# LDeakin/zarrs_tools

Hardware: AMD Instinct MI355X
Metric: GiB/s filtered (device-resident), guided_filter r=4, 2048³ f32, 256³ chunks (higher is better)
Workload: dtype f32; 1 GPU; guided_filter eps=2500 r=4 on a 2048x2048x2048 f32 array, 256^3 chunks, device-resident; rank g owns a z-slab of chunk rows + 2r halo; chunks_total=512, chunks_rank0=512, parallelism=chunk-rows x1 (strong)

## Files before the change

### zarrs_tools_amd/csrc/gf_fused.hpp

```cpp
#pragma once

#include <hip/hip_runtime.h>

#include <atomic>
#include <stdint.h>

#include <algorithm>
#include <type_traits>

#include "zt_device.hpp"
#include "zt_kernels.hpp"

#ifndef GF_K4_R4
#define GF_K4_R4 8
#endif
#ifndef GF_ORDER_R4
#define GF_ORDER_R4 2
#endif
#ifndef GF_ORDER
#define GF_ORDER 0
#endif
#ifndef GF_PRIO
#define GF_PRIO 1
#endif
#ifndef GF_HX_B128
#define GF_HX_B128 1
#endif
#ifndef GF_P1RING_MAXR
#define GF_P1RING_MAXR 2
#endif
#ifndef GF_K3
#define GF_K3 4
#endif
#ifndef GF_K4
#define GF_K4 4
#endif
#ifndef GF_STX
#define GF_STX 4
#endif
#ifndef GF_STY
#define GF_STY 16
#endif
#ifndef GF_P1PFD
#define GF_P1PFD 2
#endif
#ifndef GF_P1PFD_R4M1
#define GF_P1PFD_R4M1 1
#endif
#ifndef GF_P1PFD_R2
#define GF_P1PFD_R2 2
#endif
#ifndef GF_CNTREG
#define GF_CNTREG 1
#endif
#ifndef GF_P3VPF
#define GF_P3VPF 2
#endif
#ifndef GF_P5VPF
#define GF_P5VPF 1
#endif
#ifndef GF_WAVE_SKIP
#define GF_WAVE_SKIP 1
#endif

namespace zt {

template <int R, int K>
__device__ __forceinline__ void tree_window_sums(const float (&in)[K + 2 * R], float (&out)[K]) {
    constexpr int W = 2 * R + 1;
    if constexpr (W == 1) {
#pragma unroll
        for (int i = 0; i < K; ++i) out[i] = in[i];
    } else {
        constexpr int N = K + 2 * R;
        float p2[N], p4[N], p8[N], p16[N], p32[N], p64[N], p128[N];
#pragma unroll
        for (int i = 0; i + 1 < N; ++i) p2[i] = in[i] + in[i + 1];
        if constexpr (W >= 4) {
#pragma unroll
            for (int i = 0; i + 3 < N; ++i) p4[i] = p2[i] + p2[i + 2];
        }
        if constexpr (W >= 8) {
#pragma unroll
            for (int i = 0; i + 7 < N; ++i) p8[i] = p4[i] + p4[i + 4];
        }
        if constexpr (W >= 16) {
#pragma unroll
            for (int i = 0; i + 15 < N; ++i) p16[i] = p8[i] + p8[i + 8];
        }
        if constexpr (W >= 32) {
#pragma unroll
            for (int i = 0; i + 31 < N; ++i) p32[i] = p16[i] + p16[i + 16];
        }
        if constexpr (W >= 64) {
#pragma unroll
            for (int i = 0; i + 63 < N; ++i) p64[i] = p32[i] + p32[i + 32];
        }
        if constexpr (W >= 128) {
#pragma unroll
            for (int i = 0; i + 127 < N; ++i) p128[i] = p64[i] + p64[i + 64];
        }
#pragma unroll
        for (int i = 0; i < K; ++i) {
            float acc = 0.0f;
            int off = 0;
            bool first = true;
#pragma unroll
            for (int b = 7; b >= 0; --b) {
                if (W & (1 << b)) {
                    float piece;
                    switch (b) {
                    case 0: piece = in[i + off]; break;
                    case 1: piece = p2[i + off]; break;
                    case 2: piece = p4[i + off]; break;
                    case 3: piece = p8[i + off]; break;
                    case 4: piece = p16[i + off]; break;
                    case 5: piece = p32[i + off]; break;
                    case 6: piece = p64[i + off]; break;
                    default: piece = p128[i + off]; break;
                    }
                    acc = first ? piece : acc + piece;
                    first = false;
                    off += 1 << b;
                }
            }
            out[i] = acc;
        }
    }
}

template <int R, int K, typename T>
__device__ __forceinline__ void tree_window_sums_t(const T (&in)[K + 2 * R], T (&out)[K]) {
    constexpr int W = 2 * R + 1;
    constexpr int N = K + 2 * R;
    if constexpr (W == 1) {
#pragma unroll
        for (int i = 0; i < K; ++i) out[i] = in[i];
    } else {
        T p2[N], p4[N], p8[N], p16[N];
#pragma unroll
        for (int i = 0; i + 1 < N; ++i) p2[i] = in[i] + in[i + 1];
        if constexpr (W >= 4) {
#pragma unroll
            for (int i = 0; i + 3 < N; ++i) p4[i] = p2[i] + p2[i + 2];
        }
        if constexpr (W >= 8) {
#pragma unroll
            for (int i = 0; i + 7 < N; ++i) p8[i] = p4[i] + p4[i + 4];
        }
        if constexpr (W >= 16) {
#pragma unroll
            for (int i = 0; i + 15 < N; ++i) p16[i] = p8[i] + p8[i + 8];
        }
        static_assert(W < 32, "fused radii only");
#pragma unroll
        for (int i = 0; i < K; ++i) {
            T acc{};
            int off = 0;
            bool first = true;
#pragma unroll
            for (int b = 4; b >= 0; --b) {
                if (W & (1 << b)) {
                    T piece;
                    switch (b) {
                    case 0: piece = in[i + off]; break;
                    case 1: piece = p2[i + off]; break;
                    case 2: piece = p4[i + off]; break;
                    case 3: piece = p8[i + off]; break;
                    default: piece = p16[i + off]; break;
                    }
                    acc = first ? piece : acc + piece;
                    first = false;
                    off += 1 << b;
                }
            }
            out[i] = acc;
        }
    }
}


typedef float f2 __attribute__((ext_vector_type(2)));

__device__ __forceinline__ f2 pk_fma(f2 a, f2 b, f2 c) { return __builtin_elementwise_fma(a, b, c); }

template <int R, int K, typename T>
__device__ __forceinline__ void core_window_sums(const T (&in)[K + 2 * R], T (&out)[K]);

__device__ __forceinline__ int clamped_count(int i, int n, int r) {
    int lo = i - r < 0 ? 0 : i - r;
    int hi = i + r > n - 1 ? n - 1 : i + r;
    return hi - lo + 1;
}
__device__ __forceinline__ int cmul(int a, int b) { return (int)__umul24((unsigned)a, (unsigned)b); }

template <int R, int K, typename T>
__device__ __forceinline__ void core_window_sums(const T (&in)[K + 2 * R], T (&out)[K]) {
    constexpr int W = 2 * R + 1;
    if constexpr (K > W || K < 2) {
        tree_window_sums_t<R, K>(in, out);
    } else {
        constexpr int NC = W - K + 1;
        T c[NC];
#pragma unroll
        for (int j = 0; j < NC; ++j) c[j] = in[K - 1 + j];
#pragma unroll
        for (int w = 1; w < NC; w *= 2) {
#pragma unroll
            for (int j = 0; j + w < NC; j += 2 * w) c[j] = c[j] + c[j + w];
        }
        const T core = c[0];
        T left[K], right[K];
        if constexpr (K >= 2) {
            left[K - 2] = in[K - 2];
#pragma unroll
            for (int i = K - 3; i >= 0; --i) left[i] = in[i] + left[i + 1];
            right[1] = in[W];
#pragma unroll
            for (int i = 2; i < K; ++i) right[i] = right[i - 1] + in[W + i - 1];
        }
        out[0] = left[0] + core;
#pragma unroll
        for (int i = 1; i < K - 1; ++i) out[i] = (left[i] + core) + right[i];
        out[K - 1] = core + right[K - 1];
    }
}

template <int B, int E, typename F>
__device__ __forceinline__ void static_for(F&& f) {
    if constexpr (B < E) {
        f(std::integral_constant<int, B>{});
        static_for<B + 1, E>(f);
    }
}

template <int S, int W>
struct RingDispatch {
    template <typename F>
    __device__ __forceinline__ static void run(int slot, F&& f) {
        if (slot == S) f(std::integral_constant<int, S>{});
        else RingDispatch<S + 1, W>::run(slot, f);
    }
};
template <int W>
struct RingDispatch<W, W> {
    template <typename F>
    __device__ __forceinline__ static void run(int, F&&) {}
};

template <int R, int K, typename T>
__device__ __forceinline__ void slide_sums_exact(const T (&in)[K + 2 * R], T (&out)[K]) {
    T c[2 * R + 1];
#pragma unroll
    for (int j = 0; j <= 2 * R; ++j) c[j] = in[j];
#pragma unroll
    for (int w = 1; w <= 2 * R; w *= 2) {
#pragma unroll
        for (int j = 0; j + w <= 2 * R; j += 2 * w) c[j] = c[j] + c[j + w];
    }
    T d[K];
#pragma unroll
    for (int i = 1; i < K; ++i) d[i] = in[i + 2 * R] - in[i - 1];
    out[0] = c[0];
#pragma unroll
    for (int i = 1; i < K; ++i) out[i] = out[i - 1] + d[i];
}

template <typename T> struct S1 {
    using acc = double;
    using in = float;
    static constexpr int HXB = 8;
};
template <> struct S1<uint8_t> { using acc = int; using in = int; static constexpr int HXB = 4; };
template <> struct S1<uint16_t> { using acc = int; using in = int; static constexpr int HXB = 4; };

__device__ __forceinline__ float fast_div(float x, float d) {
    float y = __builtin_amdgcn_rcpf(d);
    float e = __builtin_fmaf(-d, y, 1.0f);
    y = __builtin_fmaf(e, y, y);
    float q = x * y;
    float r = __builtin_fmaf(-d, q, x);
    return __builtin_fmaf(r, y, q);
}

__device__ __forceinline__ void lds_barrier() {
    __asm__ volatile("s_waitcnt lgkmcnt(0)\n\ts_barrier" ::: "memory");
}

__device__ __forceinline__ float div_by_count(float x, float d, float rcp) {
    float q = x * rcp;
    float r = __builtin_fmaf(-q, d, x);
    return __builtin_fmaf(r, rcp, q);
}

using rsrc_t = __amdgpu_buffer_rsrc_t;
#ifndef GF_OUT_AUX
#define GF_OUT_AUX 2
#endif
constexpr int kBadOff = (int)0x80000000;

__device__ __forceinline__ rsrc_t make_rsrc(const void* base, uint32_t bytes) {
    return __builtin_amdgcn_make_buffer_rsrc(const_cast<void*>(base), (short)0, (int)bytes,
                                             0x00020000);
}

template <typename T> struct Buf;
template <> struct Buf<float> {
    template <int AUX = 0>
    __device__ static float load(rsrc_t r, int off) {
        return __builtin_bit_cast(float, __builtin_amdgcn_raw_buffer_load_b32(r, off, 0, AUX));
    }
    __device__ static void store(float v, rsrc_t r, int off) {
        __builtin_amdgcn_raw_buffer_store_b32(__builtin_bit_cast(uint32_t, v), r, off, 0, GF_OUT_AUX);
    }
};
template <> struct Buf<uint16_t> {
    template <int AUX = 0>
    __device__ static float load(rsrc_t r, int off) {
        return (float)(uint16_t)__builtin_amdgcn_raw_buffer_load_b16(r, off, 0, AUX);
    }
    __device__ static int load_int(rsrc_t r, int off) {
        return (int)(uint16_t)__builtin_amdgcn_raw_buffer_load_b16(r, off, 0, 0);
    }
    __device__ static void store(uint16_t v, rsrc_t r, int off) {
        __builtin_amdgcn_raw_buffer_store_b16(v, r, off, 0, 2);
    }
};
template <> struct Buf<uint8_t> {
    template <int AUX = 0>
    __device__ static float load(rsrc_t r, int off) {
        return (float)(uint8_t)__builtin_amdgcn_raw_buffer_load_b8(r, off, 0, AUX);
    }
    __device__ static int load_int(rsrc_t r, int off) {
        return (int)(uint8_t)__builtin_amdgcn_raw_buffer_load_b8(r, off, 0, 0);
    }
    __device__ static void store(uint8_t v, rsrc_t r, int off) {
        __builtin_amdgcn_raw_buffer_store_b8(v, r, off, 0, 2);
    }
};

__device__ __forceinline__ double dpp_from_lower(double v) {
    const int lo = __builtin_amdgcn_mov_dpp(__double2loint(v), 0x138, 0xF, 0xF, true);
    const int hi = __builtin_amdgcn_mov_dpp(__double2hiint(v), 0x138, 0xF, 0xF, true);
    return __hiloint2double(hi, lo);
}
__device__ __forceinline__ double dpp_from_upper(double v) {
    const int lo = __builtin_amdgcn_mov_dpp(__double2loint(v), 0x130, 0xF, 0xF, true);
    const int hi = __builtin_amdgcn_mov_dpp(__double2hiint(v), 0x130, 0xF, 0xF, true);
    return __hiloint2double(hi, lo);
}
__device__ __forceinline__ int dpp_from_lower(int v) {
    return __builtin_amdgcn_mov_dpp(v, 0x138, 0xF, 0xF, true);
}
__device__ __forceinline__ int dpp_from_upper(int v) {
    return __builtin_amdgcn_mov_dpp(v, 0x130, 0xF, 0xF, true);
}

typedef unsigned int u32x4 __attribute__((ext_vector_type(4)));
typedef unsigned int u32x2 __attribute__((ext_vector_type(2)));

template <typename T> struct Quad;
template <> struct Quad<float> {
    template <int AUX = 0>
    __device__ static void load(rsrc_t r, int off, float (&v)[4]) {
        const u32x4 q = __builtin_amdgcn_raw_buffer_load_b128(r, off, 0, AUX);
        v[0] = __uint_as_float(q.x); v[1] = __uint_as_float(q.y);
        v[2] = __uint_as_float(q.z); v[3] = __uint_as_float(q.w);
    }
    __device__ static void store(const float (&v)[4], rsrc_t r, int off) {
        const u32x4 q = {__float_as_uint(v[0]), __float_as_uint(v[1]), __float_as_uint(v[2]),
                         __float_as_uint(v[3])};
        __builtin_amdgcn_raw_buffer_store_b128(q, r, off, 0, GF_OUT_AUX);
    }
};
template <> struct Quad<uint16_t> {
    template <int AUX = 0>
    __device__ static void load(rsrc_t r, int off, float (&v)[4]) {
        const u32x2 q = __builtin_amdgcn_raw_buffer_load_b64(r, off, 0, AUX);
        v[0] = (float)(q.x & 0xffffu); v[1] = (float)(q.x >> 16);
        v[2] = (float)(q.y & 0xffffu); v[3] = (float)(q.y >> 16);
    }
    __device__ static void load(rsrc_t r, int off, int (&v)[4]) {
        const u32x2 q = __builtin_amdgcn_raw_buffer_load_b64(r, off, 0, 0);
        v[0] = (int)(q.x & 0xffffu); v[1] = (int)(q.x >> 16);
        v[2] = (int)(q.y & 0xffffu); v[3] = (int)(q.y >> 16);
    }
    __device__ static void store(const float (&v)[4], rsrc_t r, int off) {
        const uint32_t a = (uint32_t)from_f32<uint16_t>(v[0]) | ((uint32_t)from_f32<uint16_t>(v[1]) << 16);
        const uint32_t b = (uint32_t)from_f32<uint16_t>(v[2]) | ((uint32_t)from_f32<uint16_t>(v[3]) << 16);
        __builtin_amdgcn_raw_buffer_store_b64((u32x2){a, b}, r, off, 0, 2);
    }
};
template <> struct Quad<uint8_t> {
    template <int AUX = 0>
    __device__ static void load(rsrc_t r, int off, float (&v)[4]) {
        const uint32_t q = __builtin_amdgcn_raw_buffer_load_b32(r, off, 0, AUX);
        v[0] = (float)(q & 0xffu); v[1] = (float)((q >> 8) & 0xffu);
        v[2] = (float)((q >> 16) & 0xffu); v[3] = (float)(q >> 24);
    }
    __device__ static void load(rsrc_t r, int off, int (&v)[4]) {
        const uint32_t q = __builtin_amdgcn_raw_buffer_load_b32(r, off, 0, 0);
        v[0] = (int)(q & 0xffu); v[1] = (int)((q >> 8) & 0xffu);
        v[2] = (int)((q >> 16) & 0xffu); v[3] = (int)(q >> 24);
    }
    __device__ static void store(const float (&v)[4], rsrc_t r, int off) {
        const uint32_t a = (uint32_t)from_f32<uint8_t>(v[0]) | ((uint32_t)from_f32<uint8_t>(v[1]) << 8) |
                           ((uint32_t)from_f32<uint8_t>(v[2]) << 16) | ((uint32_t)from_f32<uint8_t>(v[3]) << 24);
        __builtin_amdgcn_raw_buffer_store_b32(a, r, off, 0, 2);
    }
};

__device__ __forceinline__ int opaque(int v) {
    __asm__ volatile("" : "+v"(v));
    return v;
}

template <typename T>
__device__ __forceinline__ void load_quad_masked(rsrc_t r, int off, int mask, float (&v)[4]) {
#pragma unroll
    for (int e = 0; e < 4; ++e)
        v[e] = Buf<T>::load(r, (mask >> e) & 1 ? off + e * (int)sizeof(T) : kBadOff);
}
template <typename T>
__device__ __forceinline__ void load_quad_masked(rsrc_t r, int off, int mask, int (&v)[4]) {
#pragma unroll
    for (int e = 0; e < 4; ++e)
        v[e] = Buf<T>::load_int(r, (mask >> e) & 1 ? off + e * (int)sizeof(T) : kBadOff);
}
template <typename T>
__device__ __forceinline__ void store_quad_masked(const float (&v)[4], rsrc_t r, int off, int mask) {
#pragma unroll
    for (int e = 0; e < 4; ++e)
        Buf<T>::store(from_f32<T>(v[e]), r, (mask >> e) & 1 ? off + e * (int)sizeof(T) : kBadOff);
}

template <int R, int TY, int NT, int HXB = 8>
struct GFConfig {
    static constexpr int TX = 64;
    static constexpr int W = 2 * R + 1;
    static constexpr int HXB_ = HXB;
    static constexpr int E2X = TX + 4 * R, E2Y = TY + 4 * R;
    static constexpr int E1X = TX + 2 * R, E1Y = TY + 2 * R;
    static constexpr int p2m4(int x) { return x + ((2 - x % 4) + 4) % 4; }
    static constexpr int ph4(int x) { return (x + 3) / 4 * 4 + ((x + 3) / 4 * 4 % 8 == 0 ? 4 : 0); }
    static constexpr int PH = HXB == 8 ? p2m4(E1X) : ph4(E1X);
    static constexpr int PA = p2m4(E1X);
    static constexpr int PB = p2m4(TX);
    static constexpr bool R4 = R == 4 && TY == 32 && NT == 1024;
    static constexpr int K3 = GF_K3, K4 = R4 ? GF_K4_R4 : GF_K4;
    static constexpr int ORDER = R4 ? GF_ORDER_R4 : GF_ORDER;
    static constexpr int K5 = TX * TY / NT;
    static constexpr int S3 = (E1Y + K3 - 1) / K3;
    static constexpr int S4 = TX / K4;
    static constexpr int N3 = E1X * S3, N4 = E1Y * S4;
    static constexpr int QPL = 1;
    static constexpr int EPL = 4 * QPL;
    static constexpr int NQ1X = E2X / EPL;
    static constexpr int RPW = 64 / NQ1X;
    static constexpr int NWAVE = NT / 64;
    static constexpr int NQP1 = (E2Y + RPW * NWAVE - 1) / (RPW * NWAVE);
    static constexpr int W12 = NQP1 == 1 ? NWAVE - (E2Y + RPW - 1) / RPW : 0;
    static constexpr int NB = (R + EPL - 1) / EPL;
    static constexpr bool P1RING = R <= GF_P1RING_MAXR;
    static constexpr int NQ5 = TX / 4 * TY;
    static constexpr int W3 = W * W * W;
    static constexpr int al(int b) { return (b + 255) / 256 * 256; }
    static constexpr int SZ_HX = al((E2Y + K3) * PH * HXB);
    static constexpr int SZ_LAB = al((E1Y + 1) * PA * 8);
    static constexpr int SZ_HAB = al((E1Y + 1) * PB * 8);
    static constexpr int SZ_RCP = al((W3 + 1) * 4);
    static constexpr int OFF_HX = 0, OFF_LAB = OFF_HX + SZ_HX;
    static constexpr int OFF_HAB = OFF_LAB + SZ_LAB;
    static constexpr int OFF_RCP = OFF_HAB + SZ_HAB;
    static constexpr int LDS_BYTES = OFF_RCP + SZ_RCP;
    static constexpr int T3 = NT - N3;
    static_assert(TX * TY % NT == 0, "tile must divide evenly over the threads");
    static_assert(TY % K5 == 0, "ring segment must divide the tile height");
    static_assert(TX % K4 == 0, "P4 segment must divide the tile width");
    static_assert(N3 <= NT && N4 <= NT, "one work item per thread per phase");
    static_assert(RPW >= 1, "an E2 row fits one wave");
    static_assert(E2X % 4 == 0, "E2 rows are whole quads");
    static_assert(E2X % EPL == 0, "E2 rows are whole lane items");
    static_assert(LDS_BYTES <= 160 * 1024, "LDS budget");
};

template <int R, int TY, int NT, typename TIn, typename TOut, int MODE>
__global__ __launch_bounds__(NT) void gf3d_fused_kernel(GFParams p) {
    using C = GFConfig<R, TY, NT, S1<TIn>::HXB>;
    using SA = typename S1<TIn>::acc;
    using SI = typename S1<TIn>::in;
    constexpr bool EDGE = MODE == 2, INTERIOR = MODE == 0;
    constexpr int TX = C::TX, W = C::W;
    constexpr int K5 = C::K5;
    constexpr int ESZ = (int)sizeof(TIn), OSZ = (int)sizeof(TOut);
    extern __shared__ __attribute__((aligned(16))) char smem[];
    SA* const Hx = reinterpret_cast<SA*>(smem + C::OFF_HX);
    float2* const Lab = reinterpret_cast<float2*>(smem + C::OFF_LAB);
    float2* const Hab = reinterpret_cast<float2*>(smem + C::OFF_HAB);
    float* const rcp_tab = reinterpret_cast<float*>(smem + C::OFF_RCP);
    for (int c = threadIdx.x; c <= C::W3; c += NT) rcp_tab[c] = c > 0 ? 1.0f / (float)c : 0.0f;

    const int nwg = gridDim.x;
    const int b = blockIdx.x;
    const int lid = (nwg % 8 == 0) ? (b % 8) * (nwg / 8) + b / 8 : b;
    const int gtx = INTERIOR ? p.itx1 - p.itx0 : p.tiles_x;
    const int gty = INTERIOR ? p.ity1 - p.ity0 : p.tiles_y;
    const int ntiles = gtx * gty;
    const int seg = lid / ntiles;
    int t = lid % ntiles;
    int tile_x, tile_y;
    {
        const int stx = GF_STX, sty = GF_STY;
        const int full_y = gty / sty * sty;
        const int per_srow = gtx * sty;
        if (t < full_y * gtx) {
            const int sr = t / per_srow, r = t % per_srow;
            const int full_x = gtx / stx * stx;
            if (r < full_x * sty) {
                tile_x = (r / (stx * sty)) * stx + r % stx;
                tile_y = sr * sty + (r / stx) % sty;
            } else {
                const int rr = r - full_x * sty, w = gtx - full_x;
                tile_x = full_x + rr % w;
                tile_y = sr * sty + rr / w;
            }
        } else {
            t -= full_y * gtx;
            tile_x = t % gtx;
            tile_y = full_y + t / gtx;
        }
    }
    if constexpr (INTERIOR) {
        tile_x += p.itx0;
        tile_y += p.ity0;
    } else {
        if (tile_x >= p.itx0 && tile_x < p.itx1 && tile_y >= p.ity0 && tile_y < p.ity1) return;
    }

    const int x0 = p.ox0 + tile_x * TX;
    const int y0 = p.oy0 + tile_y * TY;
    const int ox_end = p.ox0 + p.onx, oy_end = p.oy0 + p.ony;
    const int zo_begin = p.oz0 + seg * p.zseg;
    const int zo_end = min(zo_begin + p.zseg, p.oz0 + p.onz);
    const int nz = p.nz, ny = p.ny, nx = p.nx;
    const float eps = p.eps;
    const uint32_t slice_bytes = (uint32_t)((int64_t)(p.ny - 1) * p.in_sy + p.nx) * ESZ;
    const uint32_t oslice_bytes =
        (uint32_t)((int64_t)(p.ony - 1) * p.out_sy + p.onx) * OSZ;
    const int sy = (int)p.in_sy, osy = (int)p.out_sy;

    const char* in_base = static_cast<const char*>(p.in);
    const int zlo = p.zlo, zspan = p.zhi - p.zlo;
    auto slice_rsrc = [&](int z) -> rsrc_t {
        const bool ok = (unsigned)(z - zlo) < (unsigned)zspan;
        const char* base = in_base + (ok ? (int64_t)(z - p.in_z0) * p.in_sz * ESZ : 0);
        return make_rsrc(base, ok ? slice_bytes : 0u);
    };

    const int zc_begin = zo_begin - R, zc_end = zo_end + R;

    const int tid0 = threadIdx.x;
    constexpr int EPL = C::EPL;
    int q1off[C::NQP1], q1mask[C::NQP1];
    auto p12_pos = [&](int tid, int k, int& row, int& cq) -> bool {
        const int w = tid / 64 - C::W12, l = tid % 64;
        row = (k * C::NWAVE + w) * C::RPW + l / C::NQ1X;
        cq = l % C::NQ1X;
        return w >= 0 && l < C::RPW * C::NQ1X && row < C::E2Y;
    };
#pragma unroll
    for (int k = 0; k < C::NQP1; ++k) {
        int row, cq;
        const bool valid = p12_pos(tid0, k, row, cq);
        const int gx = x0 - 2 * R + EPL * cq, gy = y0 - 2 * R + row;
        int m = 0;
        if (valid && gy >= 0 && gy < ny) {
#pragma unroll
            for (int e = 0; e < 4; ++e) m |= (gx + e >= 0 && gx + e < nx) ? (1 << e) : 0;
        }
        q1mask[k] = m;
        q1off[k] = (EDGE ? valid : m == 0xF) ? (gy * sy + gx) * ESZ : kBadOff;
    }
    auto load_quad = [&](rsrc_t r, int off, int mask, SI (&v)[4]) {
        if constexpr (EDGE) load_quad_masked<TIn>(r, off, mask, v);
        else Quad<TIn>::load(r, off, v);
    };

    SA zv[C::NQP1][EPL];
#pragma unroll
    for (int k = 0; k < C::NQP1; ++k)
#pragma unroll
        for (int e = 0; e < EPL; ++e) zv[k][e] = (SA)0;
    SI ring1[C::P1RING ? W : 1][C::NQP1][EPL];
    if constexpr (C::P1RING) {
        static_for<0, W>([&](auto jc) {
            constexpr int j = decltype(jc)::value;
            const rsrc_t rs = slice_rsrc(zc_begin - 1 - R + j);
#pragma unroll
            for (int k = 0; k < C::NQP1; ++k) {
                SI v[4];
                load_quad(rs, q1off[k], q1mask[k], v);
#pragma unroll
                for (int e = 0; e < 4; ++e) {
                    ring1[(j + W - 1) % W][k][e] = v[e];
                    zv[k][e] += (SA)v[e];
                }
            }
        });
    } else {
        const int za = max(zc_begin - 1 - R, 0), zb_ = min(zc_begin - 1 + R, nz - 1);
        for (int z = za; z <= zb_; ++z) {
            const rsrc_t rs = slice_rsrc(z);
#pragma unroll
            for (int k = 0; k < C::NQP1; ++k) {
                SI v[4];
                load_quad(rs, q1off[k], q1mask[k], v);
#pragma unroll
                for (int e = 0; e < 4; ++e) zv[k][e] += (SA)v[e];
            }
        }
    }

    f2 ring[W][K5], pre[K5];
#pragma unroll
    for (int s = 0; s < W; ++s)
#pragma unroll
        for (int j = 0; j < K5; ++j) ring[s][j] = (f2){0.0f, 0.0f};
#pragma unroll
    for (int j = 0; j < K5; ++j) pre[j] = (f2){0.0f, 0.0f};

    constexpr bool R4M1 = C::R4 && MODE == 1;
    constexpr int PF = EDGE ? 1 : R4M1 ? GF_P1PFD_R4M1 : R == 4 ? GF_P1PFD : R <= 2 ? GF_P1PFD_R2 : 1;
    SI pa[PF][C::NQP1][EPL], ps[PF][C::NQP1][EPL];
    constexpr int PF3 = R4M1 ? GF_P3VPF : 1, PF5 = R4M1 ? GF_P5VPF : 1;
    static_assert(PF <= 2 && PF3 <= 2 && PF5 <= 2, "the unroll covers one or two windows");
    float vc[PF3][C::K3];
    float v5[PF5][K5];
#pragma unroll
    for (int b = 0; b < PF5; ++b)
#pragma unroll
        for (int j = 0; j < K5; ++j) v5[b][j] = 0.0f;
    constexpr bool CNTREG = R4M1 && GF_CNTREG;
    constexpr int NP3 = C::K3 / 2;
    f2 fc3[NP3], rc3[NP3];
    float rc5[K5];
    bool ok3[C::K3];
#pragma unroll
    for (int k = 0; k < NP3; ++k) fc3[k] = rc3[k] = (f2){0.0f, 0.0f};
#pragma unroll
    for (int j = 0; j < K5; ++j) rc5[j] = 0.0f;
    if constexpr (CNTREG) {
        const int item = tid0 - C::T3;
        const int gx = x0 - R + item % C::E1X, gy0 = y0 - R + item / C::E1X * C::K3;
#pragma unroll
        for (int k = 0; k < C::K3; ++k)
            ok3[k] = item >= 0 && gx >= 0 && gx < nx && gy0 + k >= 0 && gy0 + k < ny;
    }
    auto load_p1 = [&](auto bc, rsrc_t ra, rsrc_t rs) {
        constexpr int b = decltype(bc)::value;
#pragma unroll
        for (int k = 0; k < C::NQP1; ++k) {
            SI a4[4], s4[4];
            load_quad(ra, q1off[k], q1mask[k], a4);
            if constexpr (!C::P1RING) load_quad(rs, q1off[k], q1mask[k], s4);
#pragma unroll
            for (int e = 0; e < 4; ++e) {
                pa[b][k][e] = a4[e];
                if constexpr (!C::P1RING) ps[b][k][e] = s4[e];
            }
        }
    };
    auto do_p12 = [&](int tid, auto slotc, auto bc) {
        constexpr int sl = decltype(slotc)::value;
        constexpr int b = decltype(bc)::value;
#pragma unroll
        for (int k = 0; k < C::NQP1; ++k) {
            int row, cq;
            const bool valid = p12_pos(tid, k, row, cq);
#pragma unroll
            for (int e = 0; e < EPL; ++e) {
                zv[k][e] = zv[k][e] + (SA)pa[b][k][e];
                if constexpr (C::P1RING) {
                    zv[k][e] = zv[k][e] - (SA)ring1[sl][k][e];
                    ring1[sl][k][e] = pa[b][k][e];
                } else {
                    zv[k][e] = zv[k][e] - (SA)ps[b][k][e];
                }
            }
            constexpr int NB = C::NB;
            SA win[EPL * (2 * NB + 1)];
#pragma unroll
            for (int e = 0; e < EPL; ++e) win[EPL * NB + e] = zv[k][e];
#pragma unroll
            for (int n = 1; n <= NB; ++n)
#pragma unroll
                for (int e = 0; e < EPL; ++e) {
                    win[EPL * (NB - n) + e] = dpp_from_lower(win[EPL * (NB - n + 1) + e]);
                    win[EPL * (NB + n) + e] = dpp_from_upper(win[EPL * (NB + n - 1) + e]);
                }
            SA vin[EPL + 2 * R], hs[EPL];
#pragma unroll
            for (int j = 0; j < EPL + 2 * R; ++j) vin[j] = win[EPL * NB - R + j];
            slide_sums_exact<R, EPL>(vin, hs);
            if constexpr (C::HXB_ == 4 && R % 4 == 0) {
                const int col4 = EPL * cq - R;
                if (valid && col4 >= 0 && col4 + 3 < C::E1X)
                    *reinterpret_cast<int4*>(Hx + row * C::PH + col4) =
                        make_int4(hs[0], hs[1], hs[2], hs[3]);
            } else if constexpr (C::HXB_ == 4 && R % 2 == 0) {
#pragma unroll
                for (int h = 0; h < EPL / 2; ++h) {
                    const int colh = EPL * cq + 2 * h - R;
                    if (valid && colh >= 0 && colh + 1 < C::E1X)
                        *reinterpret_cast<int2*>(Hx + row * C::PH + colh) =
                            make_int2(hs[2 * h], hs[2 * h + 1]);
                }
            } else if constexpr (C::HXB_ == 8 && GF_HX_B128 && R % 2 == 0) {
#pragma unroll
                for (int h = 0; h < EPL / 2; ++h) {
                    const int colh = EPL * cq + 2 * h - R;
                    if (valid && colh >= 0 && colh + 1 < C::E1X)
                        *reinterpret_cast<double2*>(Hx + row * C::PH + colh) =
                            make_double2(hs[2 * h], hs[2 * h + 1]);
                }
            } else {
#pragma unroll
                for (int e = 0; e < EPL; ++e) {
                    const int col = EPL * cq + e - R;
                    if (valid && col >= 0 && col < C::E1X) Hx[row * C::PH + col] = hs[e];
                }
            }
        }
    };
    auto pointwise = [&](const f2 (&Uf)[NP3], const f2 (&v)[NP3], const f2 (&fc)[NP3],
                         const f2 (&rc)[NP3], f2 (&a)[NP3], f2 (&bb)[NP3]) {
        f2 q[NP3], r[NP3], u[NP3], sq[NP3], den[NP3], y[NP3], e[NP3];
#pragma unroll
        for (int k = 0; k < NP3; ++k) q[k] = Uf[k] * rc[k];
#pragma unroll
        for (int k = 0; k < NP3; ++k) r[k] = pk_fma(-q[k], fc[k], Uf[k]);
#pragma unroll
        for (int k = 0; k < NP3; ++k) u[k] = pk_fma(r[k], rc[k], q[k]);
#pragma unroll
        for (int k = 0; k < NP3; ++k) sq[k] = v[k] - u[k];
#pragma unroll
        for (int k = 0; k < NP3; ++k) sq[k] = sq[k] * sq[k];
#pragma unroll
        for (int k = 0; k < NP3; ++k) den[k] = sq[k] + (f2){eps, eps};
#pragma unroll
        for (int k = 0; k < NP3; ++k)
            y[k] = (f2){__builtin_amdgcn_rcpf(den[k].x), __builtin_amdgcn_rcpf(den[k].y)};
#pragma unroll
        for (int k = 0; k < NP3; ++k) q[k] = sq[k] * y[k];
#pragma unroll
        for (int k = 0; k < NP3; ++k) r[k] = pk_fma(-den[k], q[k], sq[k]);
#pragma unroll
        for (int k = 0; k < NP3; ++k) a[k] = pk_fma(r[k], y[k], q[k]);
#pragma unroll
        for (int k = 0; k < NP3; ++k) e[k] = (f2){1.0f, 1.0f} - a[k];
#pragma unroll
        for (int k = 0; k < NP3; ++k) bb[k] = e[k] * u[k];
    };
    static_assert(C::K3 % 2 == 0, "P3 works on pairs");
    constexpr bool kRowsWhole = C::E1Y % C::K3 == 0;
    auto p3_load = [&](int tid, SA (&vin)[C::K3 + 2 * R]) {
        const int item = tid - C::T3;
        if (item < 0) return;
        const int col = item % C::E1X, sg = item / C::E1X;
        const SA* src = Hx + (sg * C::K3) * C::PH + col;
#pragma unroll
        for (int j = 0; j < C::K3 + 2 * R; ++j) vin[j] = src[j * C::PH];
    };
    auto do_p3 = [&](int tid, int zc, auto vbc, const SA (&vin)[C::K3 + 2 * R]) {
        constexpr int vb = decltype(vbc)::value;
        const int item = tid - C::T3;
        if (item < 0) return;
        const int col = item % C::E1X, sg = item / C::E1X;
        SA U[C::K3];
        slide_sums_exact<R, C::K3>(vin, U);
        f2* lab = reinterpret_cast<f2*>(Lab);
        f2 Uf[NP3], vv[NP3], fc[NP3], rc[NP3], a[NP3], bb[NP3];
#pragma unroll
        for (int k = 0; k < NP3; ++k) {
            Uf[k] = (f2){(float)U[2 * k], (float)U[2 * k + 1]};
            vv[k] = (f2){vc[vb][2 * k], vc[vb][2 * k + 1]};
        }
        if constexpr (INTERIOR) {
            const bool zin = (unsigned)zc < (unsigned)nz;
            const int cnt = W * W * clamped_count(min(max(zc, 0), nz - 1), nz, R);
            const float fcs = (float)cnt, rcs = rcp_tab[cnt];
#pragma unroll
            for (int k = 0; k < NP3; ++k) {
                fc[k] = (f2){fcs, fcs};
                rc[k] = (f2){rcs, rcs};
            }
            pointwise(Uf, vv, fc, rc, a, bb);
#pragma unroll
            for (int k = 0; k < NP3; ++k) {
                const int ey = sg * C::K3 + 2 * k;
                const f2 ab0 = zin ? __builtin_shufflevector(a[k], bb[k], 0, 2) : (f2){0.f, 0.f};
                const f2 ab1 = zin ? __builtin_shufflevector(a[k], bb[k], 1, 3) : (f2){0.f, 0.f};
                if (kRowsWhole || ey < C::E1Y) lab[ey * C::PA + col] = ab0;
                if (kRowsWhole || ey + 1 < C::E1Y) lab[(ey + 1) * C::PA + col] = ab1;
            }
        } else if constexpr (CNTREG) {
            const bool zin = (unsigned)zc < (unsigned)nz;
            pointwise(Uf, vv, fc3, rc3, a, bb);
#pragma unroll
            for (int k = 0; k < NP3; ++k) {
                const int ey = sg * C::K3 + 2 * k;
                const bool ok0 = zin && ok3[2 * k], ok1 = zin && ok3[2 * k + 1];
                if (kRowsWhole || ey < C::E1Y) lab[ey * C::PA + col] = ok0 ? (f2){a[k].x, bb[k].x} : (f2){0.f, 0.f};
                if (kRowsWhole || ey + 1 < C::E1Y)
                    lab[(ey + 1) * C::PA + col] = ok1 ? (f2){a[k].y, bb[k].y} : (f2){0.f, 0.f};
            }
        } else {
            const int gx = x0 - R + col;
            const bool xzin = gx >= 0 && gx < nx && zc >= 0 && zc < nz;
            const int cxz = cmul(clamped_count(gx, nx, R), clamped_count(zc, nz, R));
#pragma unroll
            for (int k = 0; k < NP3; ++k) {
                const int gy = y0 - R + sg * C::K3 + 2 * k;
                const int c0 = cmul(clamped_count(gy, ny, R), cxz), c1 = cmul(clamped_count(gy + 1, ny, R), cxz);
                fc[k] = (f2){(float)c0, (float)c1};
                rc[k] = (f2){rcp_tab[c0], rcp_tab[c1]};
            }
            pointwise(Uf, vv, fc, rc, a, bb);
#pragma unroll
            for (int k = 0; k < NP3; ++k) {
                const int ey = sg * C::K3 + 2 * k;
                const int gy = y0 - R + ey;
                const bool ok0 = xzin && gy >= 0 && gy < ny, ok1 = xzin && gy + 1 >= 0 && gy + 1 < ny;
                if (kRowsWhole || ey < C::E1Y) lab[ey * C::PA + col] = ok0 ? (f2){a[k].x, bb[k].x} : (f2){0.f, 0.f};
                if (kRowsWhole || ey + 1 < C::E1Y)
                    lab[(ey + 1) * C::PA + col] = ok1 ? (f2){a[k].y, bb[k].y} : (f2){0.f, 0.f};
            }
        }
    };
    auto do_p4 = [&](int tid) {
        const int item = tid;
#if GF_WAVE_SKIP
        if (__builtin_amdgcn_readfirstlane(tid >> 6) * 64 >= C::N4) return;
#endif
        if (item >= C::N4) return;
        const int row = item % C::E1Y, sg = item / C::E1Y;
        const float4* src = reinterpret_cast<const float4*>(Lab + row * C::PA + sg * C::K4);
        f2 vin[C::K4 + 2 * R], vout[C::K4];
#pragma unroll
        for (int j = 0; j < (C::K4 + 2 * R) / 2; ++j) {
            const float4 f = src[j];
            vin[2 * j] = (f2){f.x, f.y};
            vin[2 * j + 1] = (f2){f.z, f.w};
        }
        if constexpr ((C::K4 + 2 * R) % 2) {
            const float2 t = Lab[row * C::PA + sg * C::K4 + C::K4 + 2 * R - 1];
            vin[C::K4 + 2 * R - 1] = (f2){t.x, t.y};
        }
        core_window_sums<R, C::K4>(vin, vout);
        float4* dst = reinterpret_cast<float4*>(Hab + row * C::PB + sg * C::K4);
#pragma unroll
        for (int j = 0; j < C::K4 / 2; ++j)
            dst[j] = make_float4(vout[2 * j].x, vout[2 * j].y, vout[2 * j + 1].x, vout[2 * j + 1].y);
    };
    rsrc_t ro5;
    auto p5_load = [&](int tid, f2 (&vin)[K5 + 2 * R]) {
        const int col5 = tid % TX, seg5 = tid / TX;
        const f2* src = reinterpret_cast<const f2*>(Hab) + (seg5 * K5) * C::PB + col5;
#pragma unroll
        for (int j = 0; j < K5 + 2 * R; ++j) vin[j] = src[j * C::PB];
    };
    auto do_p5 = [&](int tid, int zc, auto slot_c, auto vbc, const f2 (&vin)[K5 + 2 * R]) {
        constexpr int vb = decltype(vbc)::value;
        const int col5 = tid % TX, seg5 = tid / TX;
        f2 s2[K5];
        core_window_sums<R, K5>(vin, s2);
        constexpr int P = decltype(slot_c)::value;
        f2 AB[K5];
#pragma unroll
        for (int j = 0; j < K5; ++j) {
            pre[j] = (P == 0) ? s2[j] : pre[j] + s2[j];
            if constexpr (P == W - 1) AB[j] = pre[j];
            else AB[j] = ring[(P + 1) % W][j] + pre[j];
            ring[P][j] = s2[j];
        }
        if constexpr (P == W - 1) {
#pragma unroll
            for (int q = W - 2; q >= 0; --q)
#pragma unroll
                for (int j = 0; j < K5; ++j) ring[q][j] = ring[q][j] + ring[q + 1][j];
        }
        const int zo = zc - R;
        const int ox = x0 + col5, oyb = y0 + seg5 * K5;
        const int zq = min(max(zo, 0), nz - 1);
        f2 rc[K5];
        if constexpr (INTERIOR) {
            const float r = rcp_tab[W * W * clamped_count(zq, nz, R)];
#pragma unroll
            for (int j = 0; j < K5; ++j) rc[j] = (f2){r, r};
        } else if constexpr (CNTREG) {
#pragma unroll
            for (int j = 0; j < K5; ++j) rc[j] = (f2){rc5[j], rc5[j]};
        } else {
            const int cxz = cmul(clamped_count(ox, nx, R), clamped_count(zq, nz, R));
#pragma unroll
            for (int j = 0; j < K5; ++j) {
                const float r = rcp_tab[cmul(clamped_count(oyb + j, ny, R), cxz)];
                rc[j] = (f2){r, r};
            }
        }
#pragma unroll
        for (int j = 0; j < K5; ++j) {
            const f2 q = AB[j] * rc[j];
            const int oy = oyb + j;
            const float o = __fadd_rn(__fmul_rn(v5[vb][j], q.x), q.y);
            const int off = (ox < ox_end && oy < oy_end)
                                ? ((oy - p.oy0) * osy + (ox - p.ox0)) * OSZ : kBadOff;
            Buf<TOut>::store(from_f32<TOut>(o), ro5, opaque(off));
        }
    };

    auto load_p3v = [&](auto bc, rsrc_t r) {
        constexpr int b = decltype(bc)::value;
        const int item = (int)threadIdx.x - C::T3;
        const int col = item % C::E1X, sg = item / C::E1X;
        const int gx = x0 - R + col, gy0 = y0 - R + sg * C::K3;
#pragma unroll
        for (int k = 0; k < C::K3; ++k) {
            const int gy = gy0 + k;
            bool ok = item >= 0;
            if constexpr (EDGE) ok = ok && (unsigned)gx < (unsigned)nx && (unsigned)gy < (unsigned)ny;
            vc[b][k] = Buf<TIn>::load(r, opaque(ok ? (gy * sy + gx) * ESZ : kBadOff));
        }
    };
    auto load_p5v = [&](auto bc, rsrc_t r) {
        constexpr int b = decltype(bc)::value;
        const int col5 = (int)threadIdx.x % TX, seg5 = (int)threadIdx.x / TX;
        const int ox = x0 + col5, oyb = y0 + seg5 * K5;
#pragma unroll
        for (int j = 0; j < K5; ++j) {
            const int oy = oyb + j;
            const bool ok = ox < ox_end && oy < oy_end;
            v5[b][j] = Buf<TIn>::load(r, opaque(ok ? (oy * sy + ox) * ESZ : kBadOff));
        }
    };

    static_assert(!CNTREG || (W <= 15 && C::K3 + K5 + 2 <= 8), "the packed counts fit 32 bits");
    int cpk = 0;
    if constexpr (CNTREG) {
        const int item = max(tid0 - C::T3, 0);
        const int gx = min(max(x0 - R + item % C::E1X, 0), nx - 1);
        const int gy0 = y0 - R + item / C::E1X * C::K3;
        cpk = clamped_count(gx, nx, R);
#pragma unroll
        for (int k = 0; k < C::K3; ++k)
            cpk |= clamped_count(min(max(gy0 + k, 0), ny - 1), ny, R) << (4 + 4 * k);
        const int ox = min(x0 + tid0 % TX, nx - 1), oyb = y0 + tid0 / TX * K5;
        cpk |= clamped_count(ox, nx, R) << (4 + 4 * C::K3);
#pragma unroll
        for (int j = 0; j < K5; ++j)
            cpk |= clamped_count(min(oyb + j, ny - 1), ny, R) << (8 + 4 * C::K3 + 4 * j);
    }
    auto refresh_counts = [&](int zc3, int zo5) {
        const int cz3 = clamped_count(min(max(zc3, 0), nz - 1), nz, R);
        const int cz5 = clamped_count(min(max(zo5, 0), nz - 1), nz, R);
        const int pk = opaque(cpk);
        auto field = [&](int n) { return (pk >> (4 * n)) & 15; };
        const int cxz3 = cmul(field(0), cz3);
#pragma unroll
        for (int k = 0; k < NP3; ++k) {
            const int c0 = cmul(field(1 + 2 * k), cxz3), c1 = cmul(field(2 + 2 * k), cxz3);
            fc3[k] = (f2){(float)c0, (float)c1};
            rc3[k] = (f2){rcp_tab[c0], rcp_tab[c1]};
        }
        const int cxz5 = cmul(field(1 + C::K3), cz5);
#pragma unroll
        for (int j = 0; j < K5; ++j) rc5[j] = rcp_tab[cmul(field(2 + C::K3 + j), cxz5)];
    };

    using B0 = std::integral_constant<int, 0>;
    using BL = std::integral_constant<int, PF - 1>;
    load_p1(BL{}, slice_rsrc(zc_begin + R), slice_rsrc(zc_begin - R - 1));
    static_for<0, PF3>([&](auto jc) { load_p3v(jc, slice_rsrc(zc_begin + decltype(jc)::value)); });
    do_p12(tid0, std::integral_constant<int, W - 1>{}, BL{});
    load_p1(B0{}, slice_rsrc(zc_begin + 1 + R), slice_rsrc(zc_begin - R));
    if constexpr (PF == 2) load_p1(BL{}, slice_rsrc(zc_begin + 2 + R), slice_rsrc(zc_begin + 1 - R));
    lds_barrier();

    const int64_t sstride = p.in_sz * ESZ, osstride = p.out_sz * OSZ;
    const int64_t off_a = (int64_t)(2 * R + 1) * sstride;
    int zb = zc_begin + 1 - R;
    int64_t ob = (int64_t)(zb - p.in_z0) * sstride;
    int zs = zc_begin - 1 - R;
    int64_t os = (int64_t)(zs - p.oz0) * osstride;
    const char* out_base = static_cast<const char*>(p.out);
    const unsigned nzo = (unsigned)(zo_end - zo_begin);
    auto rs_in = [&](int64_t off, int z) {
        return make_rsrc(in_base + off, (unsigned)(z - zlo) < (unsigned)zspan ? slice_bytes : 0u);
    };

    constexpr int UN = std::max({PF, PF3, PF5}) * W;
    const int n_steps = (zc_end - zc_begin + 1 + UN - 1) / UN * UN;
    bool blk_full = false;
    for (int i0 = zc_begin; i0 < zc_begin + n_steps; i0 += UN) {
        const bool was_full = blk_full;
        blk_full = i0 - 1 - R >= R && i0 + UN - 1 < nz - R;
        static_for<0, UN>([&](auto kc) {
            constexpr int k = decltype(kc)::value;
            const int i = i0 + k;
            const int tid = threadIdx.x;
            if constexpr (CNTREG) {
                if (k == 0 ? !(blk_full && was_full) : !blk_full) refresh_counts(i, i - 1 - R);
            }
            const rsrc_t r_b = rs_in(ob, zb);
            ro5 = make_rsrc(out_base + os, (unsigned)(zs - zo_begin) < nzo ? oslice_bytes : 0u);
            if constexpr (GF_PRIO) __builtin_amdgcn_s_setprio(3);
            SA vin3[C::K3 + 2 * R];
            p3_load(tid, vin3);
            do_p3(tid, i, std::integral_constant<int, k % PF3>{}, vin3);
            if constexpr (GF_PRIO) __builtin_amdgcn_s_setprio(1);
            f2 vin5[K5 + 2 * R];
            p5_load(tid, vin5);
            do_p5(tid, i - 1, std::integral_constant<int, (k + W - 1) % W>{},
                  std::integral_constant<int, k % PF5>{}, vin5);
            lds_barrier();
            if constexpr (GF_PRIO) __builtin_amdgcn_s_setprio(3);
            load_p3v(std::integral_constant<int, k % PF3>{},
                     rs_in(ob + (int64_t)(R + PF3 - 1) * sstride, zb + R + PF3 - 1));
            load_p5v(std::integral_constant<int, k % PF5>{},
                     rs_in(ob + (int64_t)(PF5 - 2) * sstride, zb + PF5 - 2));
            if constexpr (C::ORDER & 2) do_p4(tid);
            using BK = std::integral_constant<int, k % PF>;
            do_p12(tid, std::integral_constant<int, k % W>{}, BK{});
            if constexpr (PF == 2)
                load_p1(BK{}, rs_in(ob + off_a + sstride, zb + 2 * R + 2), rs_in(ob + sstride, zb + 1));
            else
                load_p1(BK{}, rs_in(ob + off_a, zb + 2 * R + 1), r_b);
            if constexpr (GF_PRIO) __builtin_amdgcn_s_setprio(1);
            if constexpr (!(C::ORDER & 2)) do_p4(tid);
            lds_barrier();
            ++zb;
            ob += sstride;
            ++zs;
            os += osstride;
        });
    }
}

template <typename K>
inline std::atomic<uint64_t>& attr_devices() {
    static std::atomic<uint64_t> mask{0};
    return mask;
}
inline hipError_t allow_dynamic_lds(const void* kern, int bytes, std::atomic<uint64_t>& mask) {
    int dev = 0;
    if (hipError_t e = hipGetDevice(&dev)) return e;
    const uint64_t bit = 1ull << (dev & 63);
    if (mask.load(std::memory_order_relaxed) & bit) return hipSuccess;
    if (hipError_t e = hipFuncSetAttribute(kern, hipFuncAttributeMaxDynamicSharedMemorySize, bytes))
        return e;
    mask.fetch_or(bit, std::memory_order_relaxed);
    return hipSuccess;
}

template <int R, int TY, int NT, typename TIn, typename TOut, int MODE>
inline hipError_t launch_fused_variant(const GFParams& p, long long nwg, hipStream_t stream) {
    using C = GFConfig<R, TY, NT, S1<TIn>::HXB>;
    const size_t lds = (size_t)C::LDS_BYTES;
    auto kern = gf3d_fused_kernel<R, TY, NT, TIn, TOut, MODE>;
    if (hipError_t e = allow_dynamic_lds((const void*)kern, (int)lds, attr_devices<decltype(kern)>()))
        return e;
    if (nwg <= 0) return hipSuccess;
    if (nwg > 0x7FFFFFFFLL) return hipErrorInvalidValue;
    hipLaunchKernelGGL(kern, dim3((unsigned)nwg), dim3(NT), lds, stream, p);
    return hipGetLastError();
}

template <int R, int NT, typename TIn, typename TOut>
inline hipError_t launch_fused_cfg(const GFParams& p0, const FusedPlan& pl, hipStream_t stream) {
    constexpr int TY = fused_tile_y(R);
    using C = GFConfig<R, TY, NT>;
    static_assert(C::TX == kFusedTileX, "the plan's tile width is the kernel's");
    GFParams p = p0;
    {
        const float w3 = (float)(C::W3);
        volatile float one = 1.0f;
        p.rcp_w3 = one / w3;
    }
    p.zseg = pl.zseg;
    p.tiles_x = pl.tiles_x;
    p.tiles_y = pl.tiles_y;
    p.nseg = pl.nseg;
    p.itx0 = pl.itx0;
    p.itx1 = pl.itx1;
    p.ity0 = pl.ity0;
    p.ity1 = pl.ity1;
    const long long n_all = (long long)p.tiles_x * p.tiles_y;
    if (pl.mode1) {
        return launch_fused_variant<R, TY, NT, TIn, TOut, 1>(p, n_all * p.nseg, stream);
    }
    const long long n_int = (long long)(p.itx1 - p.itx0) * (p.ity1 - p.ity0);
    hipError_t e = hipSuccess;
    if (n_int > 0)
        e = launch_fused_variant<R, TY, NT, TIn, TOut, 0>(p, n_int * p.nseg, stream);
    if (e == hipSuccess && n_all > n_int)
        e = launch_fused_variant<R, TY, NT, TIn, TOut, 2>(p, n_all * p.nseg, stream);
    return e;
}

inline bool fused_fast_dtype(int d) { return d == kF32 || d == kU16 || d == kU8 || d == kBool; }

#define ZT_FUSED_PAIRS(R, NT)                                                                     \
    hipError_t launch_fused_radius_##R(const GFParams& p, const FusedPlan& pl, int din, int dout, \
                                       hipStream_t s) {                                           \
        auto pick_out = [&](auto tin) -> hipError_t {                                             \
            using TI = decltype(tin);                                                             \
            switch (dout) {                                                                       \
            case kF32: return launch_fused_cfg<R, NT, TI, float>(p, pl, s);                       \
            case kU16: return launch_fused_cfg<R, NT, TI, uint16_t>(p, pl, s);                    \
            case kU8: case kBool: return launch_fused_cfg<R, NT, TI, uint8_t>(p, pl, s);          \
            default: return hipErrorInvalidValue;                                                 \
            }                                                                                     \
        };                                                                                        \
        switch (din) {                                                                            \
        case kF32: return pick_out(float{});                                                      \
        case kU16: return pick_out(uint16_t{});                                                   \
        case kU8: case kBool: return pick_out(uint8_t{});                                         \
        default: return hipErrorInvalidValue;                                                     \
        }                                                                                         \
    }

}
```

Baseline: 1121 GiB/s.

## Reuse stage-1 leaving slice from LDS for output pass instead of reloading

In the radius-4 interior mode, the input values leaving the z-window in the stage-1 sliding sum are also written to a new LDS buffer. The output stage then reads its guide values from LDS instead of issuing separate global buffer loads for that slice. This removes one global read stream per slice at the cost of extra LDS space and LDS stores. Output store offsets are also precomputed into registers once, and opaque scalar barriers are added on the slab pointers to steer register allocation, which may raise register pressure.

```diff
diff --git a/zarrs_tools_amd/csrc/gf_fused.hpp b/zarrs_tools_amd/csrc/gf_fused.hpp
--- a/zarrs_tools_amd/csrc/gf_fused.hpp
+++ b/zarrs_tools_amd/csrc/gf_fused.hpp
@@ -58,6 +58,12 @@
 #endif
 #ifndef GF_P5VPF
 #define GF_P5VPF 1
+#endif
+#ifndef GF_V5LEAVE
+#define GF_V5LEAVE 1
+#endif
+#ifndef GF_P5OFFREG
+#define GF_P5OFFREG 1
 #endif
 #ifndef GF_WAVE_SKIP
 #define GF_WAVE_SKIP 1
@@ -412,6 +418,11 @@
 
 __device__ __forceinline__ int opaque(int v) {
     __asm__ volatile("" : "+v"(v));
+    return v;
+}
+
+__device__ __forceinline__ int64_t opaque_s(int64_t v) {
+    __asm__ volatile("" : "+s"(v));
     return v;
 }
 
@@ -472,7 +483,11 @@
     static constexpr int OFF_HX = 0, OFF_LAB = OFF_HX + SZ_HX;
     static constexpr int OFF_HAB = OFF_LAB + SZ_LAB;
     static constexpr int OFF_RCP = OFF_HAB + SZ_HAB;
-    static constexpr int LDS_BYTES = OFF_RCP + SZ_RCP;
+    static constexpr bool V5L = GF_V5LEAVE && R4 && R % 2 == 0 && !P1RING;
+    static constexpr int PV = TX;
+    static constexpr int SZ_VS = V5L ? al(TY * PV * 4) : 0;
+    static constexpr int OFF_VS = OFF_RCP + SZ_RCP;
+    static constexpr int LDS_BYTES = OFF_VS + SZ_VS;
     static constexpr int T3 = NT - N3;
     static_assert(TX * TY % NT == 0, "tile must divide evenly over the threads");
     static_assert(TY % K5 == 0, "ring segment must divide the tile height");
@@ -498,6 +513,8 @@
     float2* const Lab = reinterpret_cast<float2*>(smem + C::OFF_LAB);
     float2* const Hab = reinterpret_cast<float2*>(smem + C::OFF_HAB);
     float* const rcp_tab = reinterpret_cast<float*>(smem + C::OFF_RCP);
+    SI* const Vs = reinterpret_cast<SI*>(smem + C::OFF_VS);
+    static_assert(sizeof(SI) == 4, "Vs holds 4-byte stage-1 values");
     for (int c = threadIdx.x; c <= C::W3; c += NT) rcp_tab[c] = c > 0 ? 1.0f / (float)c : 0.0f;
 
     const int nwg = gridDim.x;
@@ -581,6 +598,16 @@
         q1mask[k] = m;
         q1off[k] = (EDGE ? valid : m == 0xF) ? (gy * sy + gx) * ESZ : kBadOff;
     }
+    constexpr bool V5LEAVE = C::V5L && MODE == 1;
+    int vs_dst[C::NQP1];
+#pragma unroll
+    for (int k = 0; k < (V5LEAVE ? C::NQP1 : 0); ++k) {
+        int row, cq;
+        const bool valid = p12_pos(tid0, k, row, cq);
+        const int ty = row - 2 * R, tq = cq - R / 2;
+        const bool in_tile = valid && (unsigned)ty < (unsigned)TY && (unsigned)tq < (unsigned)(TX / 4);
+        vs_dst[k] = opaque(in_tile ? ty * C::PV + 4 * tq : -1);
+    }
     auto load_quad = [&](rsrc_t r, int off, int mask, SI (&v)[4]) {
         if constexpr (EDGE) load_quad_masked<TIn>(r, off, mask, v);
         else Quad<TIn>::load(r, off, v);
@@ -632,7 +659,8 @@
     constexpr bool R4M1 = C::R4 && MODE == 1;
     constexpr int PF = EDGE ? 1 : R4M1 ? GF_P1PFD_R4M1 : R == 4 ? GF_P1PFD : R <= 2 ? GF_P1PFD_R2 : 1;
     SI pa[PF][C::NQP1][EPL], ps[PF][C::NQP1][EPL];
-    constexpr int PF3 = R4M1 ? GF_P3VPF : 1, PF5 = R4M1 ? GF_P5VPF : 1;
+    constexpr bool P5OFFREG = R4M1 && GF_P5OFFREG;
+    constexpr int PF3 = R4M1 ? GF_P3VPF : 1, PF5 = V5LEAVE ? 1 : R4M1 ? GF_P5VPF : 1;
     static_assert(PF <= 2 && PF3 <= 2 && PF5 <= 2, "the unroll covers one or two windows");
     float vc[PF3][C::K3];
     float v5[PF5][K5];
@@ -686,6 +714,12 @@
                 } else {
                     zv[k][e] = zv[k][e] - (SA)ps[b][k][e];
                 }
+            }
+            if constexpr (V5LEAVE) {
+                typedef SI si4 __attribute__((ext_vector_type(4)));
+                if (vs_dst[k] >= 0)
+                    *reinterpret_cast<si4*>(Vs + vs_dst[k]) =
+                        (si4){ps[b][k][0], ps[b][k][1], ps[b][k][2], ps[b][k][3]};
             }
             constexpr int NB = C::NB;
             SA win[EPL * (2 * NB + 1)];
@@ -869,8 +903,20 @@
 #pragma unroll
         for (int j = 0; j < K5 + 2 * R; ++j) vin[j] = src[j * C::PB];
     };
-    auto do_p5 = [&](int tid, int zc, auto slot_c, auto vbc, const f2 (&vin)[K5 + 2 * R]) {
+    auto p5_v = [&](int tid, auto vbc, float (&vv)[K5]) {
         constexpr int vb = decltype(vbc)::value;
+        if constexpr (V5LEAVE) {
+            const SI* src = Vs + (tid / TX * K5) * C::PV + tid % TX;
+#pragma unroll
+            for (int j = 0; j < K5; ++j) vv[j] = (float)src[j * C::PV];
+        } else {
+#pragma unroll
+            for (int j = 0; j < K5; ++j) vv[j] = v5[vb][j];
+        }
+    };
+    int off5[K5];
+    auto do_p5 = [&](int tid, int zc, auto slot_c, const float (&vv)[K5],
+                     const f2 (&vin)[K5 + 2 * R]) {
         const int col5 = tid % TX, seg5 = tid / TX;
         f2 s2[K5];
         core_window_sums<R, K5>(vin, s2);
@@ -912,12 +958,23 @@
         for (int j = 0; j < K5; ++j) {
             const f2 q = AB[j] * rc[j];
             const int oy = oyb + j;
-            const float o = __fadd_rn(__fmul_rn(v5[vb][j], q.x), q.y);
-            const int off = (ox < ox_end && oy < oy_end)
-                                ? ((oy - p.oy0) * osy + (ox - p.ox0)) * OSZ : kBadOff;
-            Buf<TOut>::store(from_f32<TOut>(o), ro5, opaque(off));
-        }
-    };
+            const float o = __fadd_rn(__fmul_rn(vv[j], q.x), q.y);
+            if constexpr (P5OFFREG) {
+                Buf<TOut>::store(from_f32<TOut>(o), ro5, off5[j]);
+            } else {
+                const int off = (ox < ox_end && oy < oy_end)
+                                    ? ((oy - p.oy0) * osy + (ox - p.ox0)) * OSZ : kBadOff;
+                Buf<TOut>::store(from_f32<TOut>(o), ro5, opaque(off));
+            }
+        }
+    };
+    if constexpr (P5OFFREG) {
+        const int ox = x0 + tid0 % TX, oyb = y0 + tid0 / TX * K5;
+#pragma unroll
+        for (int j = 0; j < K5; ++j)
+            off5[j] = opaque((ox < ox_end && oyb + j < oy_end)
+                                 ? ((oyb + j - p.oy0) * osy + (ox - p.ox0)) * OSZ : kBadOff);
+    }
 
     auto load_p3v = [&](auto bc, rsrc_t r) {
         constexpr int b = decltype(bc)::value;
@@ -1019,15 +1076,17 @@
             do_p3(tid, i, std::integral_constant<int, k % PF3>{}, vin3);
             if constexpr (GF_PRIO) __builtin_amdgcn_s_setprio(1);
             f2 vin5[K5 + 2 * R];
+            float vv5[K5];
             p5_load(tid, vin5);
-            do_p5(tid, i - 1, std::integral_constant<int, (k + W - 1) % W>{},
-                  std::integral_constant<int, k % PF5>{}, vin5);
+            p5_v(tid, std::integral_constant<int, k % PF5>{}, vv5);
+            do_p5(tid, i - 1, std::integral_constant<int, (k + W - 1) % W>{}, vv5, vin5);
             lds_barrier();
             if constexpr (GF_PRIO) __builtin_amdgcn_s_setprio(3);
             load_p3v(std::integral_constant<int, k % PF3>{},
                      rs_in(ob + (int64_t)(R + PF3 - 1) * sstride, zb + R + PF3 - 1));
-            load_p5v(std::integral_constant<int, k % PF5>{},
-                     rs_in(ob + (int64_t)(PF5 - 2) * sstride, zb + PF5 - 2));
+            if constexpr (!V5LEAVE)
+                load_p5v(std::integral_constant<int, k % PF5>{},
+                         rs_in(ob + (int64_t)(PF5 - 2) * sstride, zb + PF5 - 2));
             if constexpr (C::ORDER & 2) do_p4(tid);
             using BK = std::integral_constant<int, k % PF>;
             do_p12(tid, std::integral_constant<int, k % W>{}, BK{});
@@ -1042,6 +1101,10 @@
             ob += sstride;
             ++zs;
             os += osstride;
+            if constexpr (V5LEAVE) {
+                ob = opaque_s(ob);
+                os = opaque_s(os);
+            }
         });
     }
 }
```

New measurement: 1145 GiB/s, median of 6. 1.02x the previous value.
